# LittleWat/multichannel-semseg-with-uda

Measured on AMD Instinct MI355X. Metric: RGB-D img/s (6x480x640) MCD train step, drn_d_38, higher is better.
Workload: dtype f32 (operands split 2-way into scaled fp16, 3 cross terms on the fp16 MFMA pipe, fp32 accumulate)

## Files before the change

include/mcdseg.h:

```cpp
#ifndef MCDSEG_H
#define MCDSEG_H

#include <stddef.h>
#include <stdint.h>

#ifdef __cplusplus
extern "C" {
#endif
#pragma GCC visibility push(default)

#define MCDSEG_VERSION 101

int mcdseg_version(void);
const char* mcdseg_last_error(void);

#define MCDSEG_COMM_ID_BYTES 128
int mcdseg_comm_unique_id(void* id128);
int mcdseg_comm_init(void** comm, int32_t nranks, const void* id128, int32_t rank);
int mcdseg_comm_destroy(void* comm);
int mcdseg_allreduce(float* buf, int64_t count, void* comm, void* stream);

int32_t mcdseg_option_count(void);
const char* mcdseg_option_name(int32_t index);
int mcdseg_set_option(const char* name, int64_t value);
// ... 3 lines not shown
  int32_t N, Cin, H, W;
  int32_t Cout, KH, KW;
  int32_t stride, pad, dil;
  int32_t Ho, Wo;
  int32_t Ncb;
} mcdseg_conv_desc;

int mcdseg_conv_packed_dims(const mcdseg_conv_desc* d, int32_t* Mp_f, int32_t* Kp_f, int32_t* Mp_d, int32_t* Kp_d);
int mcdseg_conv_pack_weights(const mcdseg_conv_desc* d, const float* w, float* wp_fprop, float* wp_dgrad, void* stream);

int64_t mcdseg_conv_stat_rows(const mcdseg_conv_desc* d);
int mcdseg_conv_fprop(const mcdseg_conv_desc* d, const float* x, const float* wp_fprop, const float* bias,
                      float* y, float* stat_partials, void* stream);
int mcdseg_conv_fprop_affine(const mcdseg_conv_desc* d, const float* x, const float* wp_fprop, const float* scale,
                             const float* shift, const float* residual, int32_t relu, float* y, void* stream);
int mcdseg_conv_dgrad(const mcdseg_conv_desc* d, const float* dy, const float* wp_dgrad, float* dx, void* stream);
#define MCDSEG_MATH_F16X3 3
#define MCDSEG_MATH_BF16X6 6
#define MCDSEG_MATH_F16X1 1
int mcdseg_conv_split_packed_bytes(const mcdseg_conv_desc* d, int32_t math, int64_t* fprop_bytes, int64_t* dgrad_bytes);
int32_t mcdseg_conv_split_direct_ok(const mcdseg_conv_desc* d);
int64_t mcdseg_conv_split_stat_rows(const mcdseg_conv_desc* d);
int64_t mcdseg_conv_split_stat_rows_for(const mcdseg_conv_desc* d, int32_t math, int32_t presplit);
int32_t mcdseg_conv_split_window_ok(const mcdseg_conv_desc* d, int32_t math, int32_t presplit, int32_t dgrad);
int32_t mcdseg_conv_split_tile_config(int32_t M, int64_t P, int32_t presplit);
int mcdseg_absmax(const float* x, int64_t n, float* bound, void* stream);
int mcdseg_conv_split_pack_weights(const mcdseg_conv_desc* d, int32_t math, const float* w, void* wp_fprop, void* wp_dgrad,
                                   float* w_bound, void* stream);
int mcdseg_conv_split_pack_weights_multi(const int64_t* ptrs, const int32_t* dims, int32_t n, int32_t math, float* bounds,
                                         void* stream);
int mcdseg_conv_split_fprop(const mcdseg_conv_desc* d, int32_t math, const float* x, const void* x_cb, const float* x_bound,
                            const void* wp_fprop, const float* w_bound, const float* bias, float* y, float* stat_partials,
                            void* stream);
int mcdseg_conv_split_fprop_affine(const mcdseg_conv_desc* d, int32_t math, const float* x, const void* x_cb, const float* x_bound,
                                   const void* wp_fprop, const float* w_bound, const float* scale, const float* shift,
                                   const float* residual, int32_t relu, float* y, void* stream);
int mcdseg_conv_split_dgrad(const mcdseg_conv_desc* d, int32_t math, const float* dy, const void* dy_cb, const float* dy_bound,
                            const void* wp_dgrad, const float* w_bound, float* dx, void* stream);
int mcdseg_conv_split_dgrad_add(const mcdseg_conv_desc* d, int32_t math, const float* dy, const void* dy_cb, const float* dy_bound,
                                const void* wp_dgrad, const float* w_bound, const float* addend, float* dx, int32_t part, void* stream);
int64_t mcdseg_conv_split_parts(const mcdseg_conv_desc* d, int32_t math, int32_t presplit, int32_t dgrad);
int32_t mcdseg_conv_split_rest_pingpong(const mcdseg_conv_desc* d, int32_t math, int32_t presplit, int32_t dgrad);
int32_t mcdseg_conv_split_wide_pingpong(const mcdseg_conv_desc* d, int32_t math, int32_t presplit, int32_t dgrad);
int mcdseg_conv_split_fprop_part(const mcdseg_conv_desc* d, int32_t math, const float* x, const void* x_cb, const float* x_bound,
                                 const void* wp_fprop, const float* w_bound, const float* bias, float* y, float* stat_partials,
                                 int32_t part, void* stream);
int mcdseg_conv_split_dgrad_part(const mcdseg_conv_desc* d, int32_t math, const float* dy, const void* dy_cb, const float* dy_bound,
                                 const void* wp_dgrad, const float* w_bound, float* dx, int32_t part, void* stream);
int mcdseg_conv_split_wgrad(const mcdseg_conv_desc* d, int32_t math, const float* x, const void* x_cb, const float* x_bound,
                            const float* dy, const void* dy_cb, const float* dy_bound, float* dw, void* workspace,
                            size_t workspace_bytes, void* stream);
int32_t mcdseg_conv_wgrad_variant(const mcdseg_conv_desc* d, int32_t math, int32_t presplit);
int32_t mcdseg_conv_wgrad_fits(const mcdseg_conv_desc* d, int32_t math, int32_t presplit);
size_t mcdseg_conv_wgrad_workspace_bytes(const mcdseg_conv_desc* d);
int mcdseg_conv_wgrad(const mcdseg_conv_desc* d, const float* x, const float* dy, float* dw,
                      void* workspace, size_t workspace_bytes, void* stream);

size_t mcdseg_bn_stats_workspace_bytes(int64_t rows, int32_t C);
int mcdseg_bn_stats_finalize(const float* stat_partials, int64_t rows, int32_t C, int32_t Mp,
                             float* mean, float* rstd, float* running_mean, float* running_var,
                             int64_t* num_batches_tracked, float momentum, float eps,
                             const float* gamma, const float* beta, const float* res_bound, float* y_bound,
                             int32_t running_updates, void* workspace, size_t workspace_bytes, void* stream);
int mcdseg_bn_eval_stats(const float* running_mean, const float* running_var, int32_t C, float eps,
                         float* mean, float* rstd, void* stream);
int mcdseg_bn_eval_affine(const float* gamma, const float* beta, const float* running_mean, const float* running_var,
                          const float* conv_bias, int32_t C, float eps, float* scale, float* shift, void* stream);
int mcdseg_bn_apply(const float* z, const float* mean, const float* rstd, const float* gamma, const float* beta,
                    const float* residual, float* y, int32_t N, int32_t C, int32_t HW, int32_t relu, void* stream);
int mcdseg_split_cb(const float* x, void* x_cb, const float* x_bound, int32_t math, int32_t N, int32_t C, int32_t HW, void* stream);
int mcdseg_split_cb_padded(const float* x, void* x_cb, const float* x_bound, int32_t math, int32_t N, int32_t C, int32_t HW,
                           void* stream);
int mcdseg_unsplit_cb(const void* x_cb, const float* x_bound, int32_t math, int32_t N, int32_t C, int32_t HW, float* x, void* stream);
int mcdseg_bn_apply_cb(const float* z, const float* mean, const float* rstd, const float* gamma, const float* beta,
                       const float* residual, const void* res_cb, const float* res_bound, float* y, void* y_cb,
                       const float* y_bound, int32_t math, int32_t N, int32_t C, int32_t HW, int32_t relu, void* stream);
int mcdseg_bn_bwd_apply_cb(const float* dy, const float* y, const void* y_cb, const float* z, const float* mean, const float* rstd,
                           const float* gamma, const float* dgamma, const float* dbeta, float* dz, float* dres,
                           void* dz_cb, const float* dz_bound, int32_t math, int32_t N, int32_t C, int32_t HW, int32_t relu,
                           int32_t train, void* stream);
int mcdseg_bn_bwd_reduce_zmask(const float* dy, const float* z, const float* mean, const float* rstd, const float* gamma,
                               const float* beta, float* dgamma, float* dbeta, float* dz_bound, int32_t train, int32_t N, int32_t C,
                               int32_t HW, void* workspace, size_t workspace_bytes, void* stream);
int mcdseg_bn_bwd_apply_cb_zmask(const float* dy, const float* z, const float* mean, const float* rstd, const float* gamma,
                                 const float* beta, const float* dgamma, const float* dbeta, float* dz, void* dz_cb,
                                 const float* dz_bound, int32_t math, int32_t N, int32_t C, int32_t HW, int32_t train, void* stream);
size_t mcdseg_bn_relu_mask_bytes(int32_t N, int32_t C, int32_t HW);
int mcdseg_bn_apply_cb_mask(const float* z, const float* mean, const float* rstd, const float* gamma, const float* beta,
                            const float* residual, float* y, void* y_cb, const float* y_bound, void* relu_mask, int32_t math, int32_t N,
                            int32_t C, int32_t HW, void* stream);
int mcdseg_bn_bwd_reduce_mask(const float* dy, const void* relu_mask, const float* z, const float* mean, const float* rstd,
                              const float* gamma, float* dgamma, float* dbeta, float* dz_bound, int32_t train, int32_t N, int32_t C,
                              int32_t HW, void* workspace, size_t workspace_bytes, void* stream);
int mcdseg_bn_bwd_apply_cb_mask(const float* dy, const void* relu_mask, const float* z, const float* mean, const float* rstd,
                                const float* gamma, const float* dgamma, const float* dbeta, float* dz, float* dres, void* dz_cb,
                                const float* dz_bound, int32_t math, int32_t N, int32_t C, int32_t HW, int32_t train, void* stream);
size_t mcdseg_bn_bwd_workspace_bytes(int32_t N, int32_t C, int32_t HW);
int mcdseg_bn_bwd_reduce(const float* dy, const float* y, const void* y_cb, int32_t math, const float* z, const float* mean,
                         const float* rstd, float* dgamma, float* dbeta, const float* gamma, float* dz_bound, int32_t train,
                         int32_t N, int32_t C, int32_t HW, int32_t relu,
                         void* workspace, size_t workspace_bytes, void* stream);
int mcdseg_bn_bwd_apply(const float* dy, const float* y, const float* z, const float* mean, const float* rstd,
                        const float* gamma, const float* dgamma, const float* dbeta, float* dz, float* dres,
                        int32_t N, int32_t C, int32_t HW, int32_t relu, int32_t train, void* stream);

int mcdseg_up8_fwd(const float* x, const float* w, const float* x2, const float* w2, float* y,
// ... 102 lines not shown
```

multichannel-semseg-with-uda_amd/csrc/conv_wgrad_split_pp.hip:

```cpp
#include <cstdlib>
#include <type_traits>

#include "split.h"

namespace {

struct WgradPpParams {
  const void* x_cb;
  const void* dy_cb;
  float* slab;
  int N, Cin, H, W, Cout, Ho, Wo;
  int KH, KW, stride, pad, dil;
  int co_tiles, ci_tiles;
  int tiles_x, tiles_y;
  int kt;
  int L, nwg;
  int slabs;
  int items;
  int x_cb_bytes, dy_cb_bytes;
  long long x_piece_stride, dy_piece_stride;
};

template <class P>
__global__ __launch_bounds__(512) void conv_wgrad_split_pp_kernel(WgradPpParams p) {
  static_assert(P::NP == 2, "two-piece policies");
  constexpr int WM = 4, WN = 2;
  constexpr int NP = P::NP;
  constexpr int NBLK = 2;
  typedef typename P::frag frag;
  typedef short s16x4 __attribute__((ext_vector_type(4)));
  typedef short s16x8 __attribute__((ext_vector_type(8)));
  constexpr int NDMA = 4;
  constexpr int DSTR = 1024 + 64;
  constexpr int BLKB = NDMA * DSTR;
  constexpr int UNIT = NBLK * BLKB;
  constexpr int STAGE = 2 * NP * UNIT;
  constexpr int NS = 3;
  static_assert(NS * STAGE <= 160 * 1024, "LDS");
  constexpr bool DEEP = P::KDEEP == 2 && P::NPU == 1 && NP == 2;
  constexpr int PRO = DEEP ? 4 : 2;
  __shared__ __attribute__((aligned(16))) unsigned char smem[NS * STAGE];

  const int t = threadIdx.x;
  const int lane = t & 63;
  const int wave = __builtin_amdgcn_readfirstlane(t >> 6);
  const int grp_id = wave >> 2;
  const int wm = grp_id, wn = wave & 3;
  const int l31 = lane & 31, lh = lane >> 5;
  const int T_ = p.KH * p.KW;

  const int w_id = (blockIdx.x & 7) * (gridDim.x >> 3) + (blockIdx.x >> 3);
  if (w_id >= p.nwg) return;
  const int tiles_all = p.co_tiles * p.ci_tiles * T_;
  const long long total = (long long)tiles_all * p.kt;
  long long g_next = (long long)w_id * p.L;
  long long g_end = g_next + p.L;
  if (g_end > total) g_end = total;
  int item = w_id;
  if (p.slabs > 0) {
    g_next = 0;
    g_end = item < p.items ? 1 : 0;
  }

  const int opnd = wave >> 2;
  const int piece = (wave >> 1) & 1;
  const int blk = wave & 1;
  const bool isx = opnd == 1;
  const int px = lane & 15;
  const int cgl = lane >> 4;
  const int sH = isx ? p.H : p.Ho;
  const int sW = isx ? p.W : p.Wo;
  const int sS = isx ? p.stride : 1;
  const int sC8 = (isx ? p.Cin : p.Cout) >> 3;
  const int sHW = sH * sW;
  const int bias = p.pad * 16 + 16;
  const char* sptr = (const char*)(isx ? p.x_cb : p.dy_cb) + piece * (isx ? p.x_piece_stride : p.dy_piece_stride) - bias;
  const int sbytes = (isx ? p.x_cb_bytes : p.dy_cb_bytes) + bias;
  const __amdgpu_buffer_rsrc_t rs = __builtin_amdgcn_make_buffer_rsrc((void*)sptr, 0, sbytes, 0x00020000);
  constexpr unsigned OOB = 0x80000000u;
  const int lane_x = px * sS;
  unsigned char* const unit_lds = smem + (opnd * NP + piece) * UNIT + blk * BLKB;
  const bool dma_on = piece < P::NPU;
  const int ntiles = p.tiles_x * p.tiles_y;

  const int gl = lane & 15;
  const int tq = gl >> 2, tpp = gl & 3;
  const int trow = ((((lane >> 4) & 1) * 2 + (tpp >> 1)) * DSTR) + tq * 16 + 8 * (tpp & 1) + (2 * lh) * 64;
  const int a_lane = wm * BLKB + trow;
  const int b_lane = (wn >> 1) * BLKB + (wn & 1) * 512 + trow;

  auto tr_read_at = [&](unsigned base, auto off_c) -> s16x4 {
    s16x4 v;
#if defined(__HIP_DEVICE_COMPILE__)
    asm volatile("ds_read_b64_tr_b16 %0, %1 offset:%2" : "=v"(v) : "v"(base), "n"(decltype(off_c)::value) : "memory");
#else
    (void)base;
    v = s16x4{};
#endif
    return v;
  };
  auto frag_of = [&](unsigned base, auto lo_c, auto hi_c) -> frag {
    const s16x4 lo = tr_read_at(base, lo_c);
    const s16x4 hi = tr_read_at(base, hi_c);
    const s16x8 v = {lo[0], lo[1], lo[2], lo[3], hi[0], hi[1], hi[2], hi[3]};
    return __builtin_bit_cast(frag, v);
  };
#if defined(__HIP_DEVICE_COMPILE__)
  const unsigned smem_lds = (unsigned)(size_t)(__attribute__((address_space(3))) unsigned char*)smem;
#else
  const unsigned smem_lds = 0;
#endif
// ... 214 lines not shown
      int k = s0;
      for (; k + 7 <= s1; k += 8, src += 8 * SL) {
        const float v0 = src[0], v1 = src[SL], v2 = src[2 * SL], v3 = src[3 * SL];
        const float v4 = src[4 * SL], v5 = src[5 * SL], v6 = src[6 * SL], v7 = src[7 * SL];
        s += (double)v0;
        s += (double)v1;
        s += (double)v2;
        s += (double)v3;
        s += (double)v4;
        s += (double)v5;
        s += (double)v6;
        s += (double)v7;
      }
      for (; k + 3 <= s1; k += 4, src += 4 * SL) {
        const float v0 = src[0], v1 = src[SL], v2 = src[2 * SL], v3 = src[3 * SL];
        s += (double)v0;
        s += (double)v1;
        s += (double)v2;
        s += (double)v3;
      }
      for (; k <= s1; ++k, src += SL) s += (double)*src;
    }
    stage[lane * T + tap] = (float)(s * sc);
  }
  __syncthreads();
  float* out = dw + ((size_t)co * Cin + ci0) * T;
  for (int i = threadIdx.x; i < nci * T; i += 256) out[i] = stage[i];
}

template <class P>
__global__ __launch_bounds__(512) void conv_wgrad_split_pp3_kernel(WgradPpParams p) {
  static_assert(P::NP == 2, "two-piece policies");
  constexpr int WM = 2, WN = 3;
  constexpr int NP = P::NP;
  typedef typename P::frag frag;
  typedef short s16x4 __attribute__((ext_vector_type(4)));
  typedef short s16x8 __attribute__((ext_vector_type(8)));
  constexpr int NDMA = 4;
  constexpr int DSTR = 1024 + 64;
  constexpr int BLKB = NDMA * DSTR;
  constexpr int STAGE = 8 * BLKB;
  constexpr int NS = 3;
  static_assert(NS * STAGE <= 160 * 1024, "LDS");
  __shared__ __attribute__((aligned(16))) unsigned char smem[NS * STAGE];

  const int t = threadIdx.x;
  const int lane = t & 63;
  const int wave = __builtin_amdgcn_readfirstlane(t >> 6);
  const int grp_id = wave >> 2;
  const int wm = grp_id, wn = wave & 3;
  const int l31 = lane & 31, lh = lane >> 5;

  const int w_id = (blockIdx.x & 7) * (gridDim.x >> 3) + (blockIdx.x >> 3);
  if (w_id >= p.nwg) return;
  const int tiles_all = p.co_tiles * p.ci_tiles * p.KH;

  const bool isx = wave >= 2;
  const int piece = isx ? ((wave - 2) & 1) : wave;
  const int kxs = isx ? ((wave - 2) >> 1) : 0;
  const int px = lane & 15;
  const int cgl = lane >> 4;
  const int sH = isx ? p.H : p.Ho;
  const int sW = isx ? p.W : p.Wo;
  const int sS = isx ? p.stride : 1;
  const int sC8 = (isx ? p.Cin : p.Cout) >> 3;
  const int sHW = sH * sW;
  const int bias = p.pad * 16 + 16;
  const char* sptr = (const char*)(isx ? p.x_cb : p.dy_cb) + piece * (isx ? p.x_piece_stride : p.dy_piece_stride) - bias;
  const int sbytes = (isx ? p.x_cb_bytes : p.dy_cb_bytes) + bias;
  const __amdgpu_buffer_rsrc_t rs = __builtin_amdgcn_make_buffer_rsrc((void*)sptr, 0, sbytes, 0x00020000);
  constexpr unsigned OOB = 0x80000000u;
  const int lane_x = px * sS;
  unsigned char* const unit_lds = smem + (isx ? (2 + piece * 3 + kxs) : piece) * BLKB;
  const bool dma_on = piece < P::NPU;
  const int ntiles = p.tiles_x * p.tiles_y;

  const int gl = lane & 15;
  const int tq = gl >> 2, tpp = gl & 3;
  const int trow = ((((lane >> 4) & 1) * 2 + (tpp >> 1)) * DSTR) + tq * 16 + 8 * (tpp & 1) + (2 * lh) * 64;
  const int a_lane = (wm * 2) * 256 + trow;
  int b_lane[WN];
#pragma unroll
  for (int j = 0; j < WN; ++j) {
    const int col0 = wn * 96 + j * 32;
    b_lane[j] = (2 + (col0 >> 7)) * BLKB + ((col0 & 127) >> 5) * 256 + trow;
  }

  auto tr_read_at = [&](unsigned base, auto off_c) -> s16x4 {
    s16x4 v;
#if defined(__HIP_DEVICE_COMPILE__)
    asm volatile("ds_read_b64_tr_b16 %0, %1 offset:%2" : "=v"(v) : "v"(base), "n"(decltype(off_c)::value) : "memory");
#else
    (void)base;
    v = s16x4{};
#endif
    return v;
  };
  auto frag_of = [&](unsigned base, auto lo_c, auto hi_c) -> frag {
    const s16x4 lo = tr_read_at(base, lo_c);
    const s16x4 hi = tr_read_at(base, hi_c);
    const s16x8 v = {lo[0], lo[1], lo[2], lo[3], hi[0], hi[1], hi[2], hi[3]};
    return __builtin_bit_cast(frag, v);
  };
#if defined(__HIP_DEVICE_COMPILE__)
  const unsigned smem_lds = (unsigned)(size_t)(__attribute__((address_space(3))) unsigned char*)smem;
#else
  const unsigned smem_lds = 0;
#endif

  for (int item = w_id; item < p.items; item += p.nwg) {
    const int sl = item / tiles_all;
    const int tile = item - sl * tiles_all;
    const int k0 = sl * p.L;
    const int k1 = k0 + p.L < p.kt ? k0 + p.L : p.kt;
    const int ky = tile % p.KH;
    const int tile_ci = (tile / p.KH) % p.ci_tiles;
    const int tile_co = tile / (p.KH * p.ci_tiles);
    const int shy = isx ? ky * p.dil - p.pad : 0;
    const int shx = isx ? kxs * p.dil - p.pad : 0;
    const int cg0 = (isx ? tile_ci : tile_co) * 16;
    unsigned vconst[NDMA];
#pragma unroll
    for (int d = 0; d < NDMA; ++d) vconst[d] = (cg0 + d + 4 * cgl) < sC8 ? (unsigned)((d + 4 * cgl) * sHW + px * sS) * 16u : OOB;

    int l_n = k0 / ntiles;
    int l_ty = (k0 - l_n * ntiles) / p.tiles_x;
    int l_tx = k0 - l_n * ntiles - l_ty * p.tiles_x;
    auto issue = [&](int stage) {
#if defined(__HIP_DEVICE_COMPILE__)
      if (dma_on) {
        const int sbase = (l_n * sC8 + cg0) * sHW;
        const int iy = l_ty * sS + shy;
        const int ux = l_tx * 16 * sS + shx;
        const bool colok = (unsigned)(ux + lane_x) < (unsigned)sW;
        const int soff = ((unsigned)iy < (unsigned)sH) ? (sbase + iy * sW + ux) * 16 + bias : 0x7FFFFFFF;
#pragma unroll
        for (int d = 0; d < NDMA; ++d)
          __builtin_amdgcn_raw_ptr_buffer_load_lds(rs, (__attribute__((address_space(3))) void*)(unit_lds + stage * STAGE + d * DSTR), 16,
                                                   colok ? vconst[d] : OOB, soff, 0, 0);
      }
#else
      (void)stage;
#endif
    };
    auto advance = [&]() {
      if (++l_tx == p.tiles_x) {
        l_tx = 0;
        if (++l_ty == p.tiles_y) {
          l_ty = 0;
          ++l_n;
        }
      }
    };

    f32x16 acc[WM][WN];
#pragma unroll
    for (int i = 0; i < WM; ++i)
#pragma unroll
      for (int j = 0; j < WN; ++j)
#pragma unroll
        for (int r = 0; r < 16; ++r) acc[i][j][r] = 0.f;

    const int nsteps = k1 - k0;
// ... 62 lines not shown
#pragma unroll
        for (int j = 0; j < WN; ++j) out[row * 384 + wn * 96 + j * 32 + l31] = acc[i][j][r];
      }
  }
}

__global__ __launch_bounds__(256) void wgrad_reduce_rt_kernel(const float* __restrict__ slab, float* __restrict__ dw, int Cout, int Cin, int KH,
                                                             int ci_tiles, int slabs, int tiles_all, const float* __restrict__ x_bound,
                                                             const float* __restrict__ dy_bound) {
  __shared__ float stage[64 * 33];
  const int T = KH * 3;
  const int co = blockIdx.y;
  const int ci0 = blockIdx.x * 64;
  const int lane = threadIdx.x & 63, wave = threadIdx.x >> 6;
  const int ci = ci0 + lane;
  const double sc = x_bound != nullptr ? (double)mcd_scale_of_bound(*x_bound) * (double)mcd_scale_of_bound(*dy_bound) : 1.0;
  const int nci = Cin - ci0 < 64 ? Cin - ci0 : 64;
  const size_t SL = (size_t)tiles_all * (128 * 384);
  for (int tap = wave; tap < T; tap += 4) {
    const int ky = tap / 3, kx = tap - ky * 3;
    const int tile = ((co >> 7) * ci_tiles + (ci0 >> 7)) * KH + ky;
    double s = 0.0;
    if (ci < Cin) {
      const float* src = slab + ((size_t)tile * 128 + (co & 127)) * 384 + kx * 128 + (ci & 127);
      int k = 0;
      for (; k + 8 <= slabs; k += 8, src += 8 * SL) {
        float v[8];
#pragma unroll
        for (int u = 0; u < 8; ++u) v[u] = src[u * SL];
#pragma unroll
        for (int u = 0; u < 8; ++u) s += (double)v[u];
      }
      for (; k < slabs; ++k, src += SL) s += (double)*src;
    }
    stage[lane * T + tap] = (float)(s * sc);
  }
  __syncthreads();
  float* out = dw + ((size_t)co * Cin + ci0) * T;
  for (int i = threadIdx.x; i < nci * T; i += 256) out[i] = stage[i];
}

int pp_compute_units() {
  if (mcd_opt(MCD_OPT_WGRAD_PP_CUS) > 0) return (int)mcd_opt(MCD_OPT_WGRAD_PP_CUS);
  if (mcd_opt(MCD_OPT_PP_CUS) > 0) return (int)mcd_opt(MCD_OPT_PP_CUS);
  static const int n = [] {
    int dev = 0, cus = 0;
    if (hipGetDevice(&dev) != hipSuccess || hipDeviceGetAttribute(&cus, hipDeviceAttributeMultiprocessorCount, dev) != hipSuccess || cus <= 0)
      cus = 256;
    return cus;
  }();
  return n;
}

}

int mcdseg_internal_wgrad_pp_plan(const mcdseg_conv_desc* d, int math, int* L, size_t* slab_floats, int* slabs_out) {
  if (mcd_opt(MCD_OPT_WGRAD_PP) == 0) return 0;
  const bool stream_k = mcd_opt(MCD_OPT_WGRAD_PP) == 1;
  if (slabs_out) *slabs_out = 0;
  if (mcd_storage_math(math) != MCDSEG_MATH_F16X3 || (d->Cin & 7) || (d->Cout & 7) || d->Cin < 129 || d->Cout < 129) return 0;
  const int T = d->KH * d->KW;
  if (T > 32 || d->pad > 128) return 0;
  const int64_t co_tiles = ceil_div(d->Cout, 256), ci_tiles = ceil_div(d->Cin, 256);
  if (co_tiles * 256 - d->Cout >= 128 || ci_tiles * 256 - d->Cin >= 128) return 0;
  const int64_t kt = (int64_t)d->N * ceil_div(d->Wo, 16) * d->Ho;
  const int64_t tiles = co_tiles * ci_tiles * T, total = tiles * kt;
  int64_t nwg = pp_compute_units();
  if (total < nwg * 32) return 0;
  if (!stream_k) {
    int64_t best_r = 0, best_ls = 0, best_ns = 0;
    double best_eff = 0.0;
    for (int64_t r = 1; r <= 4; ++r) {
      int64_t ns = r * nwg / tiles;
      if (ns < 1) continue;
      if (ns > kt / 32) ns = kt / 32;
      if (ns < 1) continue;
      const int64_t ls = ceil_div64(kt, ns);
      ns = ceil_div64(kt, ls);
      const double eff = (double)total / ((double)nwg * (double)(ceil_div64(ns * tiles, nwg) * ls));
      if (eff > best_eff + 0.02 || best_r == 0) best_r = r, best_ls = ls, best_ns = ns, best_eff = eff;
      if (best_eff >= 0.95) break;
    }
    if (best_r > 0 && best_eff >= 0.80) {
      const int64_t items = best_ns * tiles;
      const int64_t rounds = ceil_div64(items, nwg);
      if (L) *L = (int)best_ls;
      if (slabs_out) *slabs_out = (int)best_ns;
      if (slab_floats) *slab_floats = (size_t)items * 256 * 256;
      return (int)ceil_div64(items, rounds);
    }
  }
  const int64_t l = ceil_div64(total, nwg);
  if (l > kt) return 0;
  nwg = ceil_div64(total, l);
  if (L) *L = (int)l;
  if (slab_floats) *slab_floats = (size_t)(nwg + tiles + 1) * 256 * 256;
  return (int)nwg;
}

int mcdseg_internal_wgrad_pp_launch(const mcdseg_conv_desc* d, int math, const void* x_cb, const float* x_bound, const void* dy_cb,
                                    const float* dy_bound, float* dw, float* slab, hipStream_t st) {
  WgradPpParams p;
  int L = 0, slabs = 0;
  const int nwg = mcdseg_internal_wgrad_pp_plan(d, math, &L, nullptr, &slabs);
  MCD_REQUIRE(nwg > 0, "conv_wgrad_split_pp: the geometry has no stream-K plan");
  const int64_t xb = (int64_t)d->N * d->Cin * d->H * d->W * 2, yb = (int64_t)d->N * d->Cout * d->Ho * d->Wo * 2;
  MCD_REQUIRE(xb + 4096 < (1ll << 31) && yb + 4096 < (1ll << 31) && (d->Ncb == 0 || d->Ncb >= d->N),
              "conv_wgrad_split_pp: pre-split operands need < 2 GiB per operand piece and Ncb >= N");
  p.x_cb = x_cb; p.dy_cb = dy_cb; p.slab = slab;
  p.N = d->N; p.Cin = d->Cin; p.H = d->H; p.W = d->W; p.Cout = d->Cout; p.Ho = d->Ho; p.Wo = d->Wo;
  p.KH = d->KH; p.KW = d->KW; p.stride = d->stride; p.pad = d->pad; p.dil = d->dil;
  p.co_tiles = ceil_div(d->Cout, 256); p.ci_tiles = ceil_div(d->Cin, 256);
  p.tiles_x = ceil_div(d->Wo, 16); p.tiles_y = d->Ho;
  p.kt = d->N * p.tiles_x * p.tiles_y;
  p.L = L; p.nwg = nwg;
  p.slabs = slabs; p.items = slabs * p.co_tiles * p.ci_tiles * d->KH * d->KW;
  p.x_cb_bytes = (int)xb; p.dy_cb_bytes = (int)yb;
  p.x_piece_stride = math == MCDSEG_MATH_F16X1 ? 0 : (long long)(d->Ncb ? d->Ncb : d->N) * d->Cin * d->H * d->W * 2;
  p.dy_piece_stride = math == MCDSEG_MATH_F16X1 ? 0 : (long long)(d->Ncb ? d->Ncb : d->N) * d->Cout * d->Ho * d->Wo * 2;
  const dim3 grid((unsigned)(8 * ceil_div(nwg, 8)));
  if (math == MCDSEG_MATH_F16X1 && mcd_opt(MCD_OPT_WGRAD_PP_DEEP) != 0)
    hipLaunchKernelGGL(conv_wgrad_split_pp_kernel<SplitF16x1D>, grid, dim3(512), 0, st, p);
  else if (math == MCDSEG_MATH_F16X1)
    hipLaunchKernelGGL(conv_wgrad_split_pp_kernel<SplitF16x1>, grid, dim3(512), 0, st, p);
  else
    hipLaunchKernelGGL(conv_wgrad_split_pp_kernel<SplitF16x3>, grid, dim3(512), 0, st, p);
  MCD_LAUNCH_CHECK("conv_wgrad_split_pp");
  const int T = d->KH * d->KW;
  MCD_REQUIRE(T <= 33, "conv_wgrad_split_pp: more than 33 taps");
  hipLaunchKernelGGL(wgrad_reduce_sk_kernel, dim3((unsigned)ceil_div(d->Cin, 64), (unsigned)d->Cout), dim3(256), 0, st, (const float*)slab, dw, d->Cout,
                     d->Cin, T, p.ci_tiles, p.kt, L, slabs, p.co_tiles * p.ci_tiles * T, x_bound, dy_bound);
  MCD_LAUNCH_CHECK("wgrad_reduce_sk");
  return 0;
}

int mcdseg_internal_wgrad_pp3_plan(const mcdseg_conv_desc* d, int math, int* L, size_t* slab_floats, int* slabs_out) {
  if (mcd_opt(MCD_OPT_WGRAD_PP3) == 0) return 0;
  if (slabs_out) *slabs_out = 0;
  if (mcd_storage_math(math) != MCDSEG_MATH_F16X3 || (d->Cin & 7) || (d->Cout & 7)) return 0;
  const int lo = d->Cin < d->Cout ? d->Cin : d->Cout;
  if (lo <= 64 || (d->Cin >= 129 && d->Cout >= 129)) return 0;
  if (d->KW != 3 || d->KH > 10 || d->pad > 128) return 0;
  const int64_t co_tiles = ceil_div(d->Cout, 128), ci_tiles = ceil_div(d->Cin, 128);
  if (4 * (int64_t)d->Cout * d->Cin < 3 * (co_tiles * 128) * (ci_tiles * 128)) return 0;
  const int64_t kt = (int64_t)d->N * ceil_div(d->Wo, 16) * d->Ho;
  const int64_t tiles = co_tiles * ci_tiles * d->KH, total = tiles * kt;
  const int64_t nwg = pp_compute_units();
  if (total < nwg * 32) return 0;
  int64_t best_r = 0, best_ls = 0, best_ns = 0;
  double best_eff = 0.0;
  for (int64_t r = 1; r <= 4; ++r) {
    int64_t ns = r * nwg / tiles;
    if (ns < 1) continue;
    if (ns > kt / 32) ns = kt / 32;
    if (ns < 1) continue;
    const int64_t ls = ceil_div64(kt, ns);
    ns = ceil_div64(kt, ls);
    const double eff = (double)total / ((double)nwg * (double)(ceil_div64(ns * tiles, nwg) * ls));
    if (eff > best_eff + 0.02 || best_r == 0) best_r = r, best_ls = ls, best_ns = ns, best_eff = eff;
    if (best_eff >= 0.95) break;
  }
  if (best_r == 0 || best_eff < 0.80) return 0;
  const int64_t items = best_ns * tiles;
  const int64_t rounds = ceil_div64(items, nwg);
  if (items * 128 * 384 >= (1ll << 31)) return 0;
  if (L) *L = (int)best_ls;
  if (slabs_out) *slabs_out = (int)best_ns;
  if (slab_floats) *slab_floats = (size_t)items * 128 * 384;
  return (int)ceil_div64(items, rounds);
}

int mcdseg_internal_wgrad_pp3_launch(const mcdseg_conv_desc* d, int math, const void* x_cb, const float* x_bound, const void* dy_cb,
                                     const float* dy_bound, float* dw, float* slab, hipStream_t st) {
  WgradPpParams p;
  int L = 0, slabs = 0;
  const int nwg = mcdseg_internal_wgrad_pp3_plan(d, math, &L, nullptr, &slabs);
  MCD_REQUIRE(nwg > 0 && slabs > 0, "conv_wgrad_split_pp3: the geometry has no plan");
  const int64_t xb = (int64_t)d->N * d->Cin * d->H * d->W * 2, yb = (int64_t)d->N * d->Cout * d->Ho * d->Wo * 2;
  MCD_REQUIRE(xb + 4096 < (1ll << 31) && yb + 4096 < (1ll << 31) && (d->Ncb == 0 || d->Ncb >= d->N),
              "conv_wgrad_split_pp3: pre-split operands need < 2 GiB per operand piece and Ncb >= N");
  p.x_cb = x_cb; p.dy_cb = dy_cb; p.slab = slab;
  p.N = d->N; p.Cin = d->Cin; p.H = d->H; p.W = d->W; p.Cout = d->Cout; p.Ho = d->Ho; p.Wo = d->Wo;
  p.KH = d->KH; p.KW = d->KW; p.stride = d->stride; p.pad = d->pad; p.dil = d->dil;
  p.co_tiles = ceil_div(d->Cout, 128); p.ci_tiles = ceil_div(d->Cin, 128);
  p.tiles_x = ceil_div(d->Wo, 16); p.tiles_y = d->Ho;
  p.kt = d->N * p.tiles_x * p.tiles_y;
  p.L = L; p.nwg = nwg;
  p.slabs = slabs; p.items = slabs * p.co_tiles * p.ci_tiles * d->KH;
  p.x_cb_bytes = (int)xb; p.dy_cb_bytes = (int)yb;
  p.x_piece_stride = math == MCDSEG_MATH_F16X1 ? 0 : (long long)(d->Ncb ? d->Ncb : d->N) * d->Cin * d->H * d->W * 2;
  p.dy_piece_stride = math == MCDSEG_MATH_F16X1 ? 0 : (long long)(d->Ncb ? d->Ncb : d->N) * d->Cout * d->Ho * d->Wo * 2;
  const dim3 grid((unsigned)(8 * ceil_div(nwg, 8)));
  if (math == MCDSEG_MATH_F16X1)
    hipLaunchKernelGGL(conv_wgrad_split_pp3_kernel<SplitF16x1>, grid, dim3(512), 0, st, p);
  else
    hipLaunchKernelGGL(conv_wgrad_split_pp3_kernel<SplitF16x3>, grid, dim3(512), 0, st, p);
  MCD_LAUNCH_CHECK("conv_wgrad_split_pp3");
  hipLaunchKernelGGL(wgrad_reduce_rt_kernel, dim3((unsigned)ceil_div(d->Cin, 64), (unsigned)d->Cout), dim3(256), 0, st, (const float*)slab, dw, d->Cout,
                     d->Cin, d->KH, p.ci_tiles, slabs, p.co_tiles * p.ci_tiles * d->KH, x_bound, dy_bound);
  MCD_LAUNCH_CHECK("wgrad_reduce_rt");
  return 0;
}
```

multichannel-semseg-with-uda_amd/csrc/options.h:

```cpp
#pragma once
#include <stdint.h>

#define MCD_OPTIONS(X)                                                                                                       \
  X(BN_STATS_ONE, 1024)                     \
  X(BN_REVERSE, 1)                              \
  X(BN_V4, 1)                                         \
  X(BIGTILE_MIN_SLOTS, 1024)                               \
  X(WIDETILE_MIN_SLOTS, 1024)                                                                 \
  X(DGRAD_INTERLEAVE, 1)       \
  X(DGRAD_ADD_LDS, 1)                   \
  X(PACK_BLOCKS, 192)                               \
  X(PP_MIN_ROUNDS, 2)          \
  X(PP_CUS, 0)                 \
  X(PINGPONG, 3)               \
  X(PP_WIDE_FILL, 80)                               \
  X(PP_WIDE128, 1)                                                                                \
  X(PP_DEEP, 1)                \
  X(THIN_WINDOW, 1)                                                           \
  X(WGRAD_WGS, 1024)                                  \
  X(WGRAD_THIN_TR, 1)                                                               \
  X(WGRAD_TR64, 1)                                                    \
  X(WGRAD_BIG, 1)                                                                       \
  X(WGRAD_PP_CUS, 0)                          \
  X(WGRAD_PP, 2)                                          \
  X(WGRAD_PP3, 1)                                                                 \
  X(WGRAD_PP_DEEP, 1)          \
  X(UP8_LOSS_DMA, 1)                                  \
  X(UP8_BAND_ROWS, -1)

enum McdOpt {
#define X(name, def) MCD_OPT_##name,
  MCD_OPTIONS(X)
#undef X
      MCD_OPT_COUNT
};

int64_t mcd_opt(McdOpt which);
```

multichannel-semseg-with-uda_amd/mcdseg/_lib.py:

```python
import ctypes
import glob
import os
import subprocess
import threading

HERE = os.path.dirname(os.path.abspath(__file__))
PKG = os.path.dirname(HERE)
REPO = os.path.dirname(PKG)
CSRC = os.path.join(PKG, "csrc")
INCLUDE = os.path.join(REPO, "include")
LIB_PATH = os.environ.get("MCDSEG_LIB") or os.path.join(HERE, "libmcdseg.so")

c_void_p, c_int, c_i32, c_i64, c_float, c_size_t = (ctypes.c_void_p, ctypes.c_int, ctypes.c_int32, ctypes.c_int64,
                                                    ctypes.c_float, ctypes.c_size_t)


class ConvDesc(ctypes.Structure):
    _fields_ = [(n, c_i32) for n in ("N", "Cin", "H", "W", "Cout", "KH", "KW", "stride", "pad", "dil", "Ho", "Wo", "Ncb")]


_P = ctypes.POINTER
_SIGNATURES = {
    "mcdseg_version": (c_int, []),
    "mcdseg_last_error": (ctypes.c_char_p, []),
    "mcdseg_option_count": (c_i32, []),
    "mcdseg_option_name": (ctypes.c_char_p, [c_i32]),
    "mcdseg_set_option": (c_int, [ctypes.c_char_p, c_i64]),
    "mcdseg_get_option": (c_int, [ctypes.c_char_p, _P(c_i64), _P(c_i64)]),
    "mcdseg_comm_unique_id": (c_int, [c_void_p]),
    "mcdseg_comm_init": (c_int, [_P(c_void_p), c_i32, c_void_p, c_i32]),
    "mcdseg_comm_destroy": (c_int, [c_void_p]),
    "mcdseg_allreduce": (c_int, [c_void_p, c_i64, c_void_p, c_void_p]),
    "mcdseg_conv_packed_dims": (c_int, [_P(ConvDesc), _P(c_i32), _P(c_i32), _P(c_i32), _P(c_i32)]),
    "mcdseg_conv_pack_weights": (c_int, [_P(ConvDesc), c_void_p, c_void_p, c_void_p, c_void_p]),
    "mcdseg_conv_stat_rows": (c_i64, [_P(ConvDesc)]),
    "mcdseg_conv_split_stat_rows": (c_i64, [_P(ConvDesc)]),
    "mcdseg_conv_split_stat_rows_for": (c_i64, [_P(ConvDesc), c_i32, c_i32]),
    "mcdseg_conv_split_window_ok": (c_i32, [_P(ConvDesc), c_i32, c_i32, c_i32]),
    "mcdseg_conv_split_direct_ok": (c_i32, [_P(ConvDesc)]),
    "mcdseg_conv_split_tile_config": (c_i32, [c_i32, c_i64, c_i32]),
    "mcdseg_conv_fprop": (c_int, [_P(ConvDesc), c_void_p, c_void_p, c_void_p, c_void_p, c_void_p, c_void_p]),
    "mcdseg_conv_fprop_affine": (c_int, [_P(ConvDesc), c_void_p, c_void_p, c_void_p, c_void_p, c_void_p, c_i32, c_void_p, c_void_p]),
    "mcdseg_bn_eval_affine": (c_int, [c_void_p] * 5 + [c_i32, c_float, c_void_p, c_void_p, c_void_p]),
    "mcdseg_predict_workspace_bytes": (c_size_t, [c_i32, c_i32]),
    "mcdseg_predict_labels": (c_int, [c_void_p] * 4 + [c_i32] * 4 + [c_void_p, c_size_t, c_void_p]),
    "mcdseg_predict_up8_workspace_bytes": (c_size_t, [c_i32, c_i32]),
    "mcdseg_predict_labels_up8": (c_int, [c_void_p] * 4 + [c_i32] * 5 + [c_void_p, c_size_t, c_void_p]),
    "mcdseg_depth_image_u8": (c_int, [c_void_p, c_void_p] + [c_i32] * 4 + [c_void_p]),
    "mcdseg_absmax": (c_int, [c_void_p, c_i64, c_void_p, c_void_p]),
    "mcdseg_conv_split_packed_bytes": (c_int, [_P(ConvDesc), c_i32, _P(c_i64), _P(c_i64)]),
    "mcdseg_conv_split_pack_weights": (c_int, [_P(ConvDesc), c_i32] + [c_void_p] * 5),
    "mcdseg_conv_split_pack_weights_multi": (c_int, [c_void_p, c_void_p, c_i32, c_i32, c_void_p, c_void_p]),
    "mcdseg_conv_split_fprop": (c_int, [_P(ConvDesc), c_i32] + [c_void_p] * 9),
    "mcdseg_conv_split_fprop_affine": (c_int, [_P(ConvDesc), c_i32] + [c_void_p] * 8 + [c_i32, c_void_p, c_void_p]),
    "mcdseg_conv_split_dgrad": (c_int, [_P(ConvDesc), c_i32] + [c_void_p] * 7),
    "mcdseg_conv_split_parts": (c_i64, [_P(ConvDesc), c_i32, c_i32, c_i32]),
    "mcdseg_conv_split_rest_pingpong": (c_i32, [_P(ConvDesc), c_i32, c_i32, c_i32]),
    "mcdseg_conv_split_wide_pingpong": (c_i32, [_P(ConvDesc), c_i32, c_i32, c_i32]),
    "mcdseg_conv_split_fprop_part": (c_int, [_P(ConvDesc), c_i32] + [c_void_p] * 8 + [c_i32, c_void_p]),
    "mcdseg_conv_split_dgrad_part": (c_int, [_P(ConvDesc), c_i32] + [c_void_p] * 6 + [c_i32, c_void_p]),
    "mcdseg_conv_split_dgrad_add": (c_int, [_P(ConvDesc), c_i32] + [c_void_p] * 7 + [c_i32, c_void_p]),
    "mcdseg_split_cb": (c_int, [c_void_p, c_void_p, c_void_p, c_i32, c_i32, c_i32, c_i32, c_void_p]),
    "mcdseg_split_cb_padded": (c_int, [c_void_p, c_void_p, c_void_p, c_i32, c_i32, c_i32, c_i32, c_void_p]),
    "mcdseg_unsplit_cb": (c_int, [c_void_p, c_void_p, c_i32, c_i32, c_i32, c_i32, c_void_p, c_void_p]),
    "mcdseg_bn_apply_cb": (c_int, [c_void_p] * 11 + [c_i32] * 5 + [c_void_p]),
    "mcdseg_bn_bwd_apply_cb": (c_int, [c_void_p] * 13 + [c_i32] * 6 + [c_void_p]),
    "mcdseg_bn_bwd_reduce_zmask": (c_int, [c_void_p] * 9 + [c_i32] * 4 + [c_void_p, c_size_t, c_void_p]),
    "mcdseg_bn_bwd_apply_cb_zmask": (c_int, [c_void_p] * 11 + [c_i32] * 5 + [c_void_p]),
    "mcdseg_bn_relu_mask_bytes": (c_size_t, [c_i32] * 3),
    "mcdseg_bn_apply_cb_mask": (c_int, [c_void_p] * 10 + [c_i32] * 4 + [c_void_p]),
    "mcdseg_bn_bwd_reduce_mask": (c_int, [c_void_p] * 9 + [c_i32] * 4 + [c_void_p, c_size_t, c_void_p]),
    "mcdseg_bn_bwd_apply_cb_mask": (c_int, [c_void_p] * 12 + [c_i32] * 5 + [c_void_p]),
    "mcdseg_conv_split_wgrad": (c_int, [_P(ConvDesc), c_i32] + [c_void_p] * 8 + [c_size_t, c_void_p]),
    "mcdseg_conv_dgrad": (c_int, [_P(ConvDesc), c_void_p, c_void_p, c_void_p, c_void_p]),
    "mcdseg_conv_wgrad_variant": (c_i32, [_P(ConvDesc), c_i32, c_i32]),
    "mcdseg_conv_wgrad_fits": (c_i32, [_P(ConvDesc), c_i32, c_i32]),
    "mcdseg_conv_wgrad_workspace_bytes": (c_size_t, [_P(ConvDesc)]),
    "mcdseg_conv_wgrad": (c_int, [_P(ConvDesc), c_void_p, c_void_p, c_void_p, c_void_p, c_size_t, c_void_p]),
    "mcdseg_bn_stats_workspace_bytes": (c_size_t, [c_i64, c_i32]),
    "mcdseg_bn_stats_finalize": (c_int, [c_void_p, c_i64, c_i32, c_i32, c_void_p, c_void_p, c_void_p, c_void_p, c_void_p,
                                         c_float, c_float, c_void_p, c_void_p, c_void_p, c_void_p, c_i32, c_void_p, c_size_t, c_void_p]),
    "mcdseg_bn_eval_stats": (c_int, [c_void_p, c_void_p, c_i32, c_float, c_void_p, c_void_p, c_void_p]),
    "mcdseg_bn_apply": (c_int, [c_void_p] * 7 + [c_i32] * 4 + [c_void_p]),
    "mcdseg_bn_bwd_workspace_bytes": (c_size_t, [c_i32, c_i32, c_i32]),
    "mcdseg_bn_bwd_reduce": (c_int, [c_void_p] * 3 + [c_i32] + [c_void_p] * 7 + [c_i32] * 5 + [c_void_p, c_size_t, c_void_p]),
    "mcdseg_bn_bwd_apply": (c_int, [c_void_p] * 10 + [c_i32] * 5 + [c_void_p]),
    "mcdseg_up8_fwd": (c_int, [c_void_p] * 5 + [c_i32] * 4 + [c_void_p]),
    "mcdseg_up8_bwd_input": (c_int, [c_void_p] * 3 + [c_i32] * 4 + [c_void_p]),
    "mcdseg_up8_bwd_weight_workspace_bytes": (c_size_t, [c_i32] * 4),
    "mcdseg_up8_bwd_weight": (c_int, [c_void_p] * 3 + [c_i32] * 4 + [c_void_p, c_size_t, c_void_p]),
    "mcdseg_up8_bwd_workspace_bytes": (c_size_t, [c_i32] * 4),
    "mcdseg_up8_bwd": (c_int, [c_void_p] * 5 + [c_i32] * 4 + [c_void_p, c_size_t, c_void_p]),
    "mcdseg_loss_workspace_bytes": (c_size_t, [c_i32, c_i32]),
    "mcdseg_softmax_ce_l1": (c_int, [c_void_p] * 4 + [c_i64, c_float, c_float] + [c_void_p] * 4 + [c_i32] * 3 +
                             [c_void_p, c_size_t, c_void_p]),
    "mcdseg_up8_loss_workspace_bytes": (c_size_t, [c_i32] * 3),
    "mcdseg_up8_softmax_ce_l1": (c_int, [c_void_p] * 6 + [c_i64, c_float, c_float] + [c_void_p] * 4 + [c_i32] * 4 +
                                 [c_void_p, c_size_t, c_void_p]),
    "mcdseg_softmax_ce_dist": (c_int, [c_void_p] * 4 + [c_i64, c_float, c_float] + [c_void_p] * 4 + [c_i32] * 4 +
                               [c_void_p, c_size_t, c_void_p]),
    "mcdseg_up8_softmax_ce_dist": (c_int, [c_void_p] * 6 + [c_i64, c_float, c_float] + [c_void_p] * 4 + [c_i32] * 5 +
                                   [c_void_p, c_size_t, c_void_p]),
    "mcdseg_label_weight_sum_workspace_bytes": (c_size_t, [c_i64]),
    "mcdseg_label_weight_sum": (c_int, [c_void_p, c_void_p, c_i64, c_i32, c_i64, c_void_p, c_void_p, c_size_t, c_void_p]),
    "mcdseg_bilinear8_fwd": (c_int, [c_void_p, c_void_p] + [c_i32] * 4 + [c_void_p]),
    "mcdseg_bilinear8_bwd": (c_int, [c_void_p, c_void_p] + [c_i32] * 4 + [c_void_p]),
    "mcdseg_mse_workspace_bytes": (c_size_t, [c_i64]),
    "mcdseg_mse": (c_int, [c_void_p] * 4 + [c_i64, c_void_p, c_size_t, c_void_p]),
    "mcdseg_gate_mix_fwd": (c_int, [c_void_p] * 4 + [c_i64, c_void_p]),
    "mcdseg_gate_mix_bwd": (c_int, [c_void_p] * 7 + [c_i64, c_void_p]),
    "mcdseg_softmax_ch_fwd": (c_int, [c_void_p, c_void_p, c_i32, c_i32, c_i32, c_void_p]),
    "mcdseg_softmax_ch_bwd": (c_int, [c_void_p, c_void_p, c_void_p, c_i32, c_i32, c_i32, c_void_p]),
    "mcdseg_prob_nll_workspace_bytes": (c_size_t, [c_i32, c_i32]),
    "mcdseg_prob_nll": (c_int, [c_void_p, c_void_p, c_void_p, c_i64, c_i32, c_void_p, c_void_p, c_i32, c_i32, c_i32, c_void_p,
                                c_size_t, c_void_p]),
    "mcdseg_normalize_u8": (c_int, [c_void_p] * 4 + [c_i32] * 6 + [c_void_p]),
    "mcdseg_resize_workspace_bytes": (c_size_t, [c_i32] * 6),
    "mcdseg_resize_bilinear_u8": (c_int, [c_void_p, c_void_p] + [c_i32] * 6 + [c_void_p, c_size_t, c_void_p]),
    "mcdseg_resize_nearest_u8": (c_int, [c_void_p, c_void_p] + [c_i32] * 5 + [c_void_p, c_size_t, c_void_p]),
    "mcdseg_relabel_u8": (c_int, [c_void_p, c_void_p, c_i64, c_i32, c_i32, c_void_p]),
    "mcdseg_confusion_hist": (c_int, [c_void_p, c_void_p, c_i64, c_i32, c_void_p, c_void_p]),
    "mcdseg_scale_by_device_scalar": (c_int, [c_void_p, c_void_p, c_i64, c_void_p]),
    "mcdseg_sgd_momentum_flat": (c_int, [c_void_p, c_void_p, c_void_p, c_i64, c_float, c_float, c_float, c_float, c_void_p]),
    "mcdseg_conv_split_half_ok": (c_i32, [_P(ConvDesc), c_i32, c_i32]),
    "mcdseg_conv_split_pp_deep": (c_i32, [_P(ConvDesc), c_i32, c_i32]),
    "mcdseg_up8_loss_variant": (c_i32, [c_i32] * 5),
    "mcdseg_conv_wgrad_thin_tr_config": (c_i32, [_P(ConvDesc)]),
    "mcdseg_conv_split_fprop_half": (c_int, [_P(ConvDesc), c_i32] + [c_void_p] * 7 + [c_i32, c_void_p]),
    "mcdseg_conv_split_dgrad_half": (c_int, [_P(ConvDesc), c_i32] + [c_void_p] * 6 + [c_i32, c_void_p]),
# ... 310 lines not shown
```

Before: 82.42.

## Reorder wgrad slab work items across XCDs to improve L2 locality

Adds a host-computed permutation of split-K wgrad work items, passed in the kernel parameters, so that workgroups landing on the same XCD share a slab and contiguous Cout/Cin tiles. The goal is fewer distinct operand tiles fetched per XCD L2, judged by a simple cost model; the permutation is used only when that model beats the natural order. The permutation is cached per geometry, and WGRAD_PP now defaults to 3 to enable it. This enlarges the kernel argument block by 512 bytes and removes the early exit for out-of-range workgroups when an order is used.

```diff
diff --git a/include/mcdseg.h b/include/mcdseg.h
--- a/include/mcdseg.h
+++ b/include/mcdseg.h
@@ -79,6 +79,7 @@
                             size_t workspace_bytes, void* stream);
 int32_t mcdseg_conv_wgrad_variant(const mcdseg_conv_desc* d, int32_t math, int32_t presplit);
 int32_t mcdseg_conv_wgrad_fits(const mcdseg_conv_desc* d, int32_t math, int32_t presplit);
+int32_t mcdseg_conv_wgrad_item_order(const mcdseg_conv_desc* d, int32_t math, int32_t kind, int32_t* items, int32_t cap, int32_t* info);
 size_t mcdseg_conv_wgrad_workspace_bytes(const mcdseg_conv_desc* d);
 int mcdseg_conv_wgrad(const mcdseg_conv_desc* d, const float* x, const float* dy, float* dw,
                       void* workspace, size_t workspace_bytes, void* stream);
diff --git a/multichannel-semseg-with-uda_amd/csrc/conv_wgrad_split_pp.hip b/multichannel-semseg-with-uda_amd/csrc/conv_wgrad_split_pp.hip
--- a/multichannel-semseg-with-uda_amd/csrc/conv_wgrad_split_pp.hip
+++ b/multichannel-semseg-with-uda_amd/csrc/conv_wgrad_split_pp.hip
@@ -1,9 +1,17 @@
+#include <algorithm>
+#include <array>
 #include <cstdlib>
+#include <map>
+#include <mutex>
 #include <type_traits>
+#include <utility>
+#include <vector>
 
 #include "split.h"
 
 namespace {
+
+constexpr int PP_ORDER_SLOTS = 256;
 
 struct WgradPpParams {
   const void* x_cb;
@@ -17,8 +25,10 @@
   int L, nwg;
   int slabs;
   int items;
+  int use_order;
   int x_cb_bytes, dy_cb_bytes;
   long long x_piece_stride, dy_piece_stride;
+  unsigned short order[PP_ORDER_SLOTS];
 };
 
 template <class P>
@@ -50,13 +60,13 @@
   const int T_ = p.KH * p.KW;
 
   const int w_id = (blockIdx.x & 7) * (gridDim.x >> 3) + (blockIdx.x >> 3);
-  if (w_id >= p.nwg) return;
+  if (p.use_order == 0 && w_id >= p.nwg) return;
   const int tiles_all = p.co_tiles * p.ci_tiles * T_;
   const long long total = (long long)tiles_all * p.kt;
   long long g_next = (long long)w_id * p.L;
   long long g_end = g_next + p.L;
   if (g_end > total) g_end = total;
-  int item = w_id;
+  int item = p.use_order ? (int)p.order[w_id] : w_id;
   if (p.slabs > 0) {
     g_next = 0;
     g_end = item < p.items ? 1 : 0;
@@ -377,7 +387,7 @@
   const int l31 = lane & 31, lh = lane >> 5;
 
   const int w_id = (blockIdx.x & 7) * (gridDim.x >> 3) + (blockIdx.x >> 3);
-  if (w_id >= p.nwg) return;
+  if (p.use_order == 0 && w_id >= p.nwg) return;
   const int tiles_all = p.co_tiles * p.ci_tiles * p.KH;
 
   const bool isx = wave >= 2;
@@ -433,7 +443,7 @@
   const unsigned smem_lds = 0;
 #endif
 
-  for (int item = w_id; item < p.items; item += p.nwg) {
+  for (int item = p.use_order ? (int)p.order[w_id] : w_id; item < p.items; item += p.nwg) {
     const int sl = item / tiles_all;
     const int tile = item - sl * tiles_all;
     const int k0 = sl * p.L;
@@ -602,6 +612,114 @@
   return n;
 }
 
+struct PpOrderGeom {
+  int tiles;
+  int blk;
+  int ci_tiles;
+  int slabs;
+  int grid;
+  double w_co, w_ci;
+};
+
+double pp_order_cost(const PpOrderGeom& g, const std::vector<int>& order) {
+  const int G = g.grid / 8;
+  double cost = 0.0;
+  for (int x = 0; x < 8; ++x) {
+    std::map<int, std::pair<uint64_t, uint64_t>> parts;
+    for (int q = 0; q < G; ++q) {
+      const int item = order[x * G + q];
+      if (item < 0) continue;
+      const int tile = item % g.tiles, pair = tile / g.blk;
+      auto& m = parts[item / g.tiles];
+      m.first |= 1ull << (pair / g.ci_tiles);
+      m.second |= 1ull << (pair % g.ci_tiles);
+    }
+    for (const auto& kv : parts) cost += __builtin_popcountll(kv.second.first) * g.w_co + __builtin_popcountll(kv.second.second) * g.w_ci;
+  }
+  return cost;
+}
+
+std::vector<int> pp_natural_order(const PpOrderGeom& g) {
+  std::vector<int> order(g.grid, -1);
+  for (int w = 0; w < g.grid && w < g.slabs * g.tiles; ++w) order[w] = w;
+  return order;
+}
+
+std::vector<int> pp_xcd_order(const PpOrderGeom& g) {
+  const int G = g.grid / 8, T = g.tiles;
+  std::vector<int> order(g.grid, -1);
+  int used[8] = {0, 0, 0, 0, 0, 0, 0, 0};
+  auto place = [&](int x, int slab, int t0, int t1) {
+    for (int t = t0; t < t1; ++t) order[x * G + used[x]++] = slab * T + t;
+  };
+  struct Run { int slab, t0, t1; };
+  std::vector<Run> left;
+  const int c = T < G ? T : G;
+  int s = 0;
+  for (int j = 0; j < G / c; ++j)
+    for (int x = 0; x < 8 && s < g.slabs; ++x, ++s) {
+      place(x, s, 0, c);
+      if (c < T) left.push_back({s, c, T});
+    }
+  for (; s < g.slabs; ++s) left.push_back({s, 0, T});
+  const int co_span = g.blk * g.ci_tiles;
+  for (Run r : left)
+    while (r.t0 < r.t1) {
+      const int len = r.t1 - r.t0;
+      int fit = -1, most = 0;
+      for (int x = 0; x < 8; ++x) {
+        const int f = G - used[x];
+        if (f >= len && (fit < 0 || f < G - used[fit])) fit = x;
+        if (f > G - used[most]) most = x;
+      }
+      if (fit >= 0) {
+        place(fit, r.slab, r.t0, r.t1);
+        break;
+      }
+      const int room = G - used[most];
+      int e = (r.t0 + room) / co_span * co_span;
+      if (e <= r.t0) e = (r.t0 + room) / g.blk * g.blk;
+      if (e <= r.t0) e = r.t0 + room;
+      place(most, r.slab, r.t0, e);
+      r.t0 = e;
+    }
+  return order;
+}
+
+std::vector<int> pp_item_order(const PpOrderGeom& g, int nwg) {
+  const long long items = (long long)g.slabs * g.tiles;
+  if (mcd_opt(MCD_OPT_WGRAD_PP) != 3 || g.slabs <= 0 || items > nwg || g.grid > PP_ORDER_SLOTS || items >= 0xFFFF) return {};
+  if (g.tiles / g.blk / g.ci_tiles > 64 || g.ci_tiles > 64) return {};
+  static std::mutex mu;
+  static std::map<std::array<long long, 7>, std::vector<int>> cache;
+  const std::array<long long, 7> key = {g.tiles, g.blk, g.ci_tiles, g.slabs, g.grid, (long long)g.w_co, (long long)g.w_ci};
+  std::lock_guard<std::mutex> lock(mu);
+  auto it = cache.find(key);
+  if (it == cache.end()) {
+    std::vector<int> order = pp_xcd_order(g);
+    if (!(pp_order_cost(g, order) < pp_order_cost(g, pp_natural_order(g)))) order.clear();
+    it = cache.emplace(key, std::move(order)).first;
+  }
+  return it->second;
+}
+
+PpOrderGeom pp_order_geom(const mcdseg_conv_desc* d, int tile_ch, int blk, int slabs, int nwg) {
+  PpOrderGeom g;
+  g.ci_tiles = ceil_div(d->Cin, tile_ch);
+  g.blk = blk;
+  g.tiles = ceil_div(d->Cout, tile_ch) * g.ci_tiles * blk;
+  g.slabs = slabs;
+  g.grid = 8 * ceil_div(nwg, 8);
+  g.w_co = (double)d->Ho * d->Wo;
+  g.w_ci = (double)d->Ho * d->Wo * d->stride;
+  return g;
+}
+
+void pp_set_order(WgradPpParams& p, const std::vector<int>& order) {
+  p.use_order = order.empty() ? 0 : 1;
+  for (int w = 0; w < PP_ORDER_SLOTS; ++w) p.order[w] = !order.empty() && w < (int)order.size() && order[w] >= 0 ? (unsigned short)order[w] : 0xFFFF;
+}
+
 }
 
 int mcdseg_internal_wgrad_pp_plan(const mcdseg_conv_desc* d, int math, int* L, size_t* slab_floats, int* slabs_out) {
@@ -665,6 +783,7 @@
   p.kt = d->N * p.tiles_x * p.tiles_y;
   p.L = L; p.nwg = nwg;
   p.slabs = slabs; p.items = slabs * p.co_tiles * p.ci_tiles * d->KH * d->KW;
+  pp_set_order(p, pp_item_order(pp_order_geom(d, 256, d->KH * d->KW, slabs, nwg), nwg));
   p.x_cb_bytes = (int)xb; p.dy_cb_bytes = (int)yb;
   p.x_piece_stride = math == MCDSEG_MATH_F16X1 ? 0 : (long long)(d->Ncb ? d->Ncb : d->N) * d->Cin * d->H * d->W * 2;
   p.dy_piece_stride = math == MCDSEG_MATH_F16X1 ? 0 : (long long)(d->Ncb ? d->Ncb : d->N) * d->Cout * d->Ho * d->Wo * 2;
@@ -737,6 +856,7 @@
   p.kt = d->N * p.tiles_x * p.tiles_y;
   p.L = L; p.nwg = nwg;
   p.slabs = slabs; p.items = slabs * p.co_tiles * p.ci_tiles * d->KH;
+  pp_set_order(p, pp_item_order(pp_order_geom(d, 128, d->KH, slabs, nwg), nwg));
   p.x_cb_bytes = (int)xb; p.dy_cb_bytes = (int)yb;
   p.x_piece_stride = math == MCDSEG_MATH_F16X1 ? 0 : (long long)(d->Ncb ? d->Ncb : d->N) * d->Cin * d->H * d->W * 2;
   p.dy_piece_stride = math == MCDSEG_MATH_F16X1 ? 0 : (long long)(d->Ncb ? d->Ncb : d->N) * d->Cout * d->Ho * d->Wo * 2;
@@ -751,3 +871,25 @@
   MCD_LAUNCH_CHECK("wgrad_reduce_rt");
   return 0;
 }
+
+extern "C" int32_t mcdseg_conv_wgrad_item_order(const mcdseg_conv_desc* d, int32_t math, int32_t kind, int32_t* items, int32_t cap, int32_t* info) {
+  int L = 0, slabs = 0;
+  size_t sf = 0;
+  const int nwg = kind == 0 ? mcdseg_internal_wgrad_pp_plan(d, math, &L, &sf, &slabs) : mcdseg_internal_wgrad_pp3_plan(d, math, &L, &sf, &slabs);
+  if (nwg <= 0 || slabs <= 0) return 0;
+  const PpOrderGeom g = kind == 0 ? pp_order_geom(d, 256, d->KH * d->KW, slabs, nwg) : pp_order_geom(d, 128, d->KH, slabs, nwg);
+  std::vector<int> order = pp_item_order(g, nwg);
+  const bool xcd = !order.empty();
+  if (!xcd) {
+    order.assign(g.grid, -1);
+    for (int w = 0; w < nwg; ++w) order[w] = w;
+  }
+  if (info) {
+    info[0] = L; info[1] = slabs; info[2] = g.tiles; info[3] = d->N * ceil_div(d->Wo, 16) * d->Ho;
+    info[4] = nwg; info[5] = g.blk; info[6] = g.ci_tiles; info[7] = xcd ? 1 : 0;
+    info[8] = (int32_t)(sf / (size_t)(kind == 0 ? 256 * 256 : 128 * 384));
+  }
+  if (items)
+    for (int w = 0; w < g.grid && w < cap; ++w) items[w] = order[w];
+  return g.grid;
+}
diff --git a/multichannel-semseg-with-uda_amd/csrc/options.h b/multichannel-semseg-with-uda_amd/csrc/options.h
--- a/multichannel-semseg-with-uda_amd/csrc/options.h
+++ b/multichannel-semseg-with-uda_amd/csrc/options.h
@@ -22,7 +22,7 @@
   X(WGRAD_TR64, 1)                                                    \
   X(WGRAD_BIG, 1)                                                                       \
   X(WGRAD_PP_CUS, 0)                          \
-  X(WGRAD_PP, 2)                                          \
+  X(WGRAD_PP, 3)               \
   X(WGRAD_PP3, 1)                                                                 \
   X(WGRAD_PP_DEEP, 1)          \
   X(UP8_LOSS_DMA, 1)                                  \
diff --git a/multichannel-semseg-with-uda_amd/mcdseg/_lib.py b/multichannel-semseg-with-uda_amd/mcdseg/_lib.py
--- a/multichannel-semseg-with-uda_amd/mcdseg/_lib.py
+++ b/multichannel-semseg-with-uda_amd/mcdseg/_lib.py
@@ -75,6 +75,7 @@
     "mcdseg_conv_dgrad": (c_int, [_P(ConvDesc), c_void_p, c_void_p, c_void_p, c_void_p]),
     "mcdseg_conv_wgrad_variant": (c_i32, [_P(ConvDesc), c_i32, c_i32]),
     "mcdseg_conv_wgrad_fits": (c_i32, [_P(ConvDesc), c_i32, c_i32]),
+    "mcdseg_conv_wgrad_item_order": (c_i32, [_P(ConvDesc), c_i32, c_i32, _P(c_i32), c_i32, _P(c_i32)]),
     "mcdseg_conv_wgrad_workspace_bytes": (c_size_t, [_P(ConvDesc)]),
     "mcdseg_conv_wgrad": (c_int, [_P(ConvDesc), c_void_p, c_void_p, c_void_p, c_void_p, c_size_t, c_void_p]),
     "mcdseg_bn_stats_workspace_bytes": (c_size_t, [c_i64, c_i32]),
```

New measurement: 82.56, median of 6. Within noise of the previous version (+0.2%).
